# maxjaritz/mvpnet

Measured on AMD Instinct MI355X. Metric: chunks/sec (8192 pts, 3x160x120 views) fwd+bwd, higher is better.
Workload: dtype f32; 1 GPU; configs[2]: MVPNet lifting (unproject + pixel k-NN + gather) + FeatureAggregation + PN2SSG full train step (fwd+loss+bwd+Adam), 2D CNN replaced by a resident 64-ch feature map; cfg=mvpnet_3d_unet_resnet34_pn2ssg.yaml, chunks_per_gpu=32, points=8192, views=3x160x120, feature_channels=64, k=3, parallelism=dp1 (one process per GPU, 1 grad all-reduce/step), launch=eager, cpu_affinity=32 logical cpus of 256 (0 .. 183)

## Files before the change

mvpnet_amd/csrc/rows.hip:

```cpp
#include <algorithm>
#include "common.h"
#include "stats_reduce.h"
#include "dropout.h"

namespace {

constexpr int kRT = 256;

__device__ __forceinline__ float4 ld4(const float* p) { return *reinterpret_cast<const float4*>(p); }
__device__ __forceinline__ void st4(float* p, float4 v) { *reinterpret_cast<float4*>(p) = v; }

__global__ __launch_bounds__(kRT) void group_rows_kernel(const float* __restrict__ feat, const float* __restrict__ xyz,
                                                         const float* __restrict__ center,
                                                         const int64_t* __restrict__ idx, int N, int C, int M, int K,
                                                         int ld, float* __restrict__ out) {
  const int b = blockIdx.y;
  const int L4 = ld >> 2;
  const int64_t E = (int64_t)M * K;
  const int64_t t = (int64_t)blockIdx.x * kRT + threadIdx.x;
  const int64_t e = t / L4;
  const int c4 = (int)(t - e * L4);
  if (e >= E) return;
  const int64_t j = idx[(size_t)b * E + e];
  const bool ok = j >= 0 && j < N;
  const int c = c4 * 4;
  float4 v = make_float4(0.f, 0.f, 0.f, 0.f);
  if (c + 4 <= C) {
    if (ok) v = ld4(feat + ((size_t)b * N + j) * C + c);
  } else if (xyz && ok) {
    const int m = (int)(e / K);
    const float* p = xyz + ((size_t)b * N + j) * 3;
    const float* q = center + ((size_t)b * M + m) * 3;
    float r[4] = {0.f, 0.f, 0.f, 0.f};
#pragma unroll
    for (int i = 0; i < 4; ++i) {
      const int col = c + i - C;
      if (col >= 0 && col < 3) r[i] = p[col] - q[col];
    }
    v = make_float4(r[0], r[1], r[2], r[3]);
  }
  st4(out + ((size_t)b * E + e) * ld + c, v);
}

constexpr int kRelU = 4;
__global__ __launch_bounds__(kRT) void relation_rows_kernel(const float* __restrict__ feat, const float* __restrict__ src,
                                                            const float* __restrict__ tgt, int64_t rows, int K, int C,
                                                            float* __restrict__ out) {
  const int L4 = (C >> 2) + 1;
  const int64_t total = rows * L4;
  const int64_t t0 = (int64_t)blockIdx.x * (kRT * kRelU) + threadIdx.x;
  float4 v[kRelU];
  int64_t dst[kRelU];
#pragma unroll
  for (int u = 0; u < kRelU; ++u) {
    const int64_t t = t0 + (int64_t)u * kRT;
    dst[u] = -1;
    if (t < total) {
      const int64_t e = t / L4;
      const int c4 = (int)(t - e * L4);
      dst[u] = e * (C + 4) + c4 * 4;
      if (c4 < L4 - 1) {
        v[u] = ld4(feat + (size_t)e * C + c4 * 4);
      } else {
        const float* p = src + (size_t)e * 3;
        const float* q = tgt + (size_t)(e / K) * 3;
        const float dx = p[0] - q[0], dy = p[1] - q[1], dz = p[2] - q[2];
        v[u] = make_float4(dx, dy, dz, (dx * dx + dy * dy) + dz * dz);
      }
    }
  }
#pragma unroll
  for (int u = 0; u < kRelU; ++u)
    if (dst[u] >= 0) st4(out + dst[u], v[u]);
}

__global__ __launch_bounds__(kRT) void relation4_rows_kernel(const float* __restrict__ src, const float* __restrict__ tgt, int64_t rows, int K,
                                                             float* __restrict__ out) {
  const int64_t e = (int64_t)blockIdx.x * kRT + threadIdx.x;
  if (e >= rows) return;
  const float* p = src + (size_t)e * 3;
  const float* q = tgt + (size_t)(e / K) * 3;
  const float dx = p[0] - q[0], dy = p[1] - q[1], dz = p[2] - q[2];
  st4(out + (size_t)e * 4, make_float4(dx, dy, dz, (dx * dx + dy * dy) + dz * dz));
// ... 476 lines not shown
    const float *mm = p.mm, *ii = p.ii, *gm = p.gg, *bt = p.bb;
    float fo[4], go[4];
#pragma unroll
    for (int i = 0; i < 4; ++i) {
      const float dz = (!relu || oo[i] > 0.f) ? dd[i] : 0.f;
      float xh;
      if (fabsf(gm[i]) >= 0.05f * (1.0f + fabsf(bt[i])))
        xh = (oo[i] - bt[i]) / gm[i];
      else
        xh = (y[((size_t)g * K + a[i]) * C + c + i] - mm[i]) * ii[i];
      fo[i] = dz;
      go[i] = dz * xh;
    }
    f = make_float4(fo[0], fo[1], fo[2], fo[3]);
    gg = make_float4(go[0], go[1], go[2], go[3]);
  }
};

struct BwdMaxSel {
  const float *dout, *out, *ysel, *mean, *invstd;
  int relu;
  struct Params { float mm[4], ii[4]; };
  __device__ __forceinline__ Params params(int c) const {
    const float4 mu = ld4(mean + c), is = ld4(invstd + c);
    Params p;
    p.mm[0] = mu.x; p.mm[1] = mu.y; p.mm[2] = mu.z; p.mm[3] = mu.w;
    p.ii[0] = is.x; p.ii[1] = is.y; p.ii[2] = is.z; p.ii[3] = is.w;
    return p;
  }
  __device__ __forceinline__ void at(const Params& p, int64_t g, int c, int C, float4& f, float4& gg) const {
    const float4 d = ld4(dout + (size_t)g * C + c), o = ld4(out + (size_t)g * C + c), ys = ld4(ysel + (size_t)g * C + c);
    const float dd[4] = {d.x, d.y, d.z, d.w}, oo[4] = {o.x, o.y, o.z, o.w}, yy[4] = {ys.x, ys.y, ys.z, ys.w};
    float fo[4], go[4];
#pragma unroll
    for (int i = 0; i < 4; ++i) {
      const float dz = (!relu || oo[i] > 0.f) ? dd[i] : 0.f;
      fo[i] = dz;
      go[i] = dz * ((yy[i] - p.mm[i]) * p.ii[i]);
    }
    f = make_float4(fo[0], fo[1], fo[2], fo[3]);
    gg = make_float4(go[0], go[1], go[2], go[3]);
  }
};

__global__ __launch_bounds__(kRT) void pool_finalize_kernel(const float* __restrict__ ymax, const float* __restrict__ ymin,
                                                            const uint8_t* __restrict__ amax, const uint8_t* __restrict__ amin,
                                                            const float* __restrict__ mean, const float* __restrict__ invstd,
                                                            const float* __restrict__ gamma, const float* __restrict__ beta, int64_t G,
                                                            int C, int relu, float* __restrict__ out, uint8_t* __restrict__ arg,
                                                            float* __restrict__ ysel) {
  const int C4 = C >> 2;
  const int64_t t = (int64_t)blockIdx.x * kRT + threadIdx.x;
  const int64_t g = t / C4;
  const int c = (int)(t - g * C4) * 4;
  if (g >= G) return;
  const float4 mu = ld4(mean + c), is = ld4(invstd + c), ga = ld4(gamma + c), be = ld4(beta + c);
  const float4 hi = ld4(ymax + (size_t)g * C + c), lo = ld4(ymin + (size_t)g * C + c);
  const uchar4 ah = *reinterpret_cast<const uchar4*>(amax + (size_t)g * C + c), al = *reinterpret_cast<const uchar4*>(amin + (size_t)g * C + c);
  const float mm[4] = {mu.x, mu.y, mu.z, mu.w}, ii[4] = {is.x, is.y, is.z, is.w}, gg[4] = {ga.x, ga.y, ga.z, ga.w};
  const float bb[4] = {be.x, be.y, be.z, be.w}, hv[4] = {hi.x, hi.y, hi.z, hi.w}, lv[4] = {lo.x, lo.y, lo.z, lo.w};
  const uint8_t ha[4] = {ah.x, ah.y, ah.z, ah.w}, la[4] = {al.x, al.y, al.z, al.w};
  float o[4], ys[4];
  uint8_t ar[4];
#pragma unroll
  for (int i = 0; i < 4; ++i) {
    const bool up = gg[i] * ii[i] >= 0.f;
    ys[i] = up ? hv[i] : lv[i];
    ar[i] = up ? ha[i] : la[i];
    const float a = ((ys[i] - mm[i]) * ii[i]) * gg[i] + bb[i];
    o[i] = (relu && !(a > 0.f)) ? 0.f : a;
  }
  st4(out + (size_t)g * C + c, make_float4(o[0], o[1], o[2], o[3]));
  st4(ysel + (size_t)g * C + c, make_float4(ys[0], ys[1], ys[2], ys[3]));
  uchar4 u;
  u.x = ar[0]; u.y = ar[1]; u.z = ar[2]; u.w = ar[3];
  *reinterpret_cast<uchar4*>(arg + (size_t)g * C + c) = u;
}

struct BwdSum {
  const float *dout, *y, *mean, *invstd, *gamma, *beta;
  int K, relu;
  typedef ColParams Params;
  __device__ __forceinline__ Params params(int c) const { return load_col_params(mean, invstd, gamma, beta, c); }
  __device__ __forceinline__ void at(const Params& p, int64_t r, int c, int C, float4& f, float4& g) const {
    const float4 yy = ld4(y + (size_t)r * C + c), d = ld4(dout + (size_t)(r / K) * C + c);
    const float yv[4] = {yy.x, yy.y, yy.z, yy.w}, dd[4] = {d.x, d.y, d.z, d.w};
    float fo[4], go[4];
#pragma unroll
    for (int i = 0; i < 4; ++i) {
      const float xh = (yv[i] - p.mm[i]) * p.ii[i];
      const float dz = (!relu || xh * p.gg[i] + p.bb[i] > 0.f) ? dd[i] : 0.f;
      fo[i] = dz;
      go[i] = dz * xh;
    }
    f = make_float4(fo[0], fo[1], fo[2], fo[3]);
    g = make_float4(go[0], go[1], go[2], go[3]);
  }
};

template <typename Src>
__global__ __launch_bounds__(kRT) void colstats_kernel(Src src, int64_t R, int C, double* __restrict__ stat,
                                                       double* __restrict__ partial, int zero_stat) {
  if (zero_stat && blockIdx.x == 0)
    for (int j = threadIdx.x; j < 2 * C; j += kRT) stat[j] = 0.0;
  __shared__ double red[2][kRT][4];
  const int C4 = C >> 2;
  const int rpp = kRT / C4;
  const int c4 = threadIdx.x % C4, rg = threadIdx.x / C4;
  const int c = c4 * 4;
  const int64_t stride = (int64_t)gridDim.x * rpp;
  double ds[4] = {0, 0, 0, 0}, dq[4] = {0, 0, 0, 0};
  if (rg < rpp) {
    const typename Src::Params prm = src.params(c);
    int64_t r = (int64_t)blockIdx.x * rpp + rg;
    while (r < R) {
      float4 s = make_float4(0.f, 0.f, 0.f, 0.f), q = s;
      for (int it = 0; it < 16 && r < R; ++it, r += 4 * stride) {
        float4 f[4], g[4];
#pragma unroll
        for (int u = 0; u < 4; ++u) {
          f[u] = make_float4(0.f, 0.f, 0.f, 0.f);
          g[u] = f[u];
          if (r + u * stride < R) src.at(prm, r + u * stride, c, C, f[u], g[u]);
        }
#pragma unroll
        for (int u = 0; u < 4; ++u) {
          s.x += f[u].x; s.y += f[u].y; s.z += f[u].z; s.w += f[u].w;
          q.x += g[u].x; q.y += g[u].y; q.z += g[u].z; q.w += g[u].w;
        }
      }
      ds[0] += s.x; ds[1] += s.y; ds[2] += s.z; ds[3] += s.w;
      dq[0] += q.x; dq[1] += q.y; dq[2] += q.z; dq[3] += q.w;
    }
  }
  double* a = red[0][threadIdx.x];
  double* bq = red[1][threadIdx.x];
#pragma unroll
  for (int i = 0; i < 4; ++i) {
    a[i] = ds[i];
    bq[i] = dq[i];
  }
  __syncthreads();
  if (rg == 0) {
    double ts[4] = {0, 0, 0, 0}, tq[4] = {0, 0, 0, 0};
    for (int g = 0; g < rpp; ++g)
#pragma unroll
      for (int i = 0; i < 4; ++i) {
        ts[i] += red[0][g * C4 + c4][i];
        tq[i] += red[1][g * C4 + c4][i];
      }
    if (partial) {
      double* slot = partial + (size_t)blockIdx.x * 2 * C;
#pragma unroll
      for (int i = 0; i < 4; ++i) {
        slot[c + i] = ts[i];
        slot[C + c + i] = tq[i];
      }
    } else {
#pragma unroll
      for (int i = 0; i < 4; ++i) {
        atomicAdd(stat + c + i, ts[i]);
        atomicAdd(stat + C + c + i, tq[i]);
      }
    }
  }
}

__global__ void bn_finalize_kernel(const double* __restrict__ stat, int64_t R, int C, float eps, float momentum,
                                   float* __restrict__ mean, float* __restrict__ invstd,
                                   float* __restrict__ running_mean, float* __restrict__ running_var,
                                   int64_t* __restrict__ num_batches_tracked) {
  const int c = blockIdx.x * blockDim.x + threadIdx.x;
  if (c >= C) return;
  if (c == 0 && num_batches_tracked) *num_batches_tracked += 1;
  const double m = stat[c] / (double)R;
  double var = stat[C + c] / (double)R - m * m;
  if (var < 0.0) var = 0.0;
  mean[c] = (float)m;
  invstd[c] = (float)(1.0 / sqrt(var + (double)eps));
  if (running_mean) {
    const double unbiased = R > 1 ? var * ((double)R / (double)(R - 1)) : var;
    running_mean[c] = (float)((1.0 - momentum) * (double)running_mean[c] + momentum * m);
    running_var[c] = (float)((1.0 - momentum) * (double)running_var[c] + momentum * unbiased);
  }
}

template <bool RELU>
__global__ __launch_bounds__(kRT) void bn_act_kernel(const float* __restrict__ y, const float* __restrict__ mean,
                                                     const float* __restrict__ invstd, const float* __restrict__ gamma,
                                                     const float* __restrict__ beta, int64_t G, int K, int C,
                                                     float* __restrict__ out, uint8_t* __restrict__ arg) {
  const int C4 = C >> 2;
  const int64_t t = (int64_t)blockIdx.x * kRT + threadIdx.x;
  const int64_t g = t / C4;
  const int c = (int)(t - g * C4) * 4;
  if (g >= G) return;
  const float4 mu = ld4(mean + c), is = ld4(invstd + c), ga = ld4(gamma + c), be = ld4(beta + c);
  const bool sum = K > 1 && arg == nullptr;
  float best[4] = {-INFINITY, -INFINITY, -INFINITY, -INFINITY};
  if (sum) best[0] = best[1] = best[2] = best[3] = 0.f;
  int bk[4] = {0, 0, 0, 0};
  for (int k = 0; k < K; ++k) {
    const float4 yy = ld4(y + ((size_t)g * K + k) * C + c);
    float a[4] = {((yy.x - mu.x) * is.x) * ga.x + be.x, ((yy.y - mu.y) * is.y) * ga.y + be.y,
                  ((yy.z - mu.z) * is.z) * ga.z + be.z, ((yy.w - mu.w) * is.w) * ga.w + be.w};
#pragma unroll
    for (int i = 0; i < 4; ++i) {
      if (RELU) a[i] = a[i] > 0.f ? a[i] : 0.f;
      if (sum) {
        best[i] += a[i];
      } else if (a[i] > best[i]) {
        best[i] = a[i];
        bk[i] = k;
      }
    }
  }
  st4(out + (size_t)g * C + c, make_float4(best[0], best[1], best[2], best[3]));
  if (arg) {
    uchar4 u;
    u.x = (uint8_t)bk[0]; u.y = (uint8_t)bk[1]; u.z = (uint8_t)bk[2]; u.w = (uint8_t)bk[3];
    *reinterpret_cast<uchar4*>(arg + (size_t)g * C + c) = u;
  }
}

template <bool RELU>
__global__ __launch_bounds__(kRT) void bn_act_rows_kernel(const float* __restrict__ y, const float* __restrict__ mean,
                                                          const float* __restrict__ invstd, const float* __restrict__ gamma,
                                                          const float* __restrict__ beta, int64_t R, int C, float* __restrict__ out,
                                                          Dropout drop) {
  const int C4 = C >> 2;
  const int64_t t = (int64_t)blockIdx.x * kRT + threadIdx.x;
  const int64_t rg = t / C4;
  const int c = (int)(t - rg * C4) * 4;
  const int64_t r0 = rg * 8;
  if (r0 >= R) return;
  const float4 mu = ld4(mean + c), is = ld4(invstd + c), ga = ld4(gamma + c), be = ld4(beta + c);
#pragma unroll
  for (int h = 0; h < 8; h += 4) {
    float4 yy[4];
#pragma unroll
    for (int u = 0; u < 4; ++u) yy[u] = (r0 + h + u < R) ? ld4(y + (size_t)(r0 + h + u) * C + c) : make_float4(0.f, 0.f, 0.f, 0.f);
#pragma unroll
    for (int u = 0; u < 4; ++u) {
      if (r0 + h + u >= R) break;
      float a[4] = {((yy[u].x - mu.x) * is.x) * ga.x + be.x, ((yy[u].y - mu.y) * is.y) * ga.y + be.y,
                    ((yy[u].z - mu.z) * is.z) * ga.z + be.z, ((yy[u].w - mu.w) * is.w) * ga.w + be.w};
      if (RELU) {
#pragma unroll
        for (int i = 0; i < 4; ++i) a[i] = a[i] > 0.f ? a[i] : 0.f;
      }
      if (drop.thresh) {
        const unsigned e = (unsigned)((r0 + h + u) * C + c);
#pragma unroll
        for (int i = 0; i < 4; ++i) a[i] *= drop.factor(e + i);
      }
      st4(out + (size_t)(r0 + h + u) * C + c, make_float4(a[0], a[1], a[2], a[3]));
    }
  }
}

constexpr int kBwdRows = 8;
template <bool RELU>
__global__ __launch_bounds__(kRT) void bn_rows_bwd_kernel(const float* __restrict__ dsrc, const float* __restrict__ y,
                                                          const float* __restrict__ mean, const float* __restrict__ invstd,
                                                          const float* __restrict__ gamma, const float* __restrict__ beta,
                                                          const double* __restrict__ stat, int64_t R, int C, int batch_terms,
                                                          float* __restrict__ dy, float* __restrict__ dgamma,
                                                          float* __restrict__ dbeta, Dropout drop) {
  const int C4 = C >> 2;
  if (blockIdx.x == 0 && dgamma)
    for (int j = threadIdx.x; j < C; j += kRT) {
      dbeta[j] = (float)stat[j];
      dgamma[j] = (float)stat[C + j];
    }
  const int64_t t = (int64_t)blockIdx.x * kRT + threadIdx.x;
  const int64_t rg = t / C4;
  const int c = (int)(t - rg * C4) * 4;
  const int64_t r0 = rg * kBwdRows;
  if (r0 >= R) return;
  const float4 mu = ld4(mean + c), is = ld4(invstd + c), ga = ld4(gamma + c), be = ld4(beta + c);
  const float mm[4] = {mu.x, mu.y, mu.z, mu.w}, ii[4] = {is.x, is.y, is.z, is.w};
  const float gg[4] = {ga.x, ga.y, ga.z, ga.w}, bb[4] = {be.x, be.y, be.z, be.w};
  const float invR = batch_terms ? 1.0f / (float)R : 0.f;
  float sc[4], db[4], dg[4];
#pragma unroll
  for (int i = 0; i < 4; ++i) {
    sc[i] = gg[i] * ii[i];
    db[i] = (float)stat[c + i] * invR;
    dg[i] = (float)stat[C + c + i] * invR;
  }
#pragma unroll
  for (int h = 0; h < kBwdRows; h += 4) {
    float4 yy[4], dd[4];
#pragma unroll
    for (int u = 0; u < 4; ++u) {
      const int64_t r = r0 + h + u;
// ... 577 lines not shown
```

mvpnet_amd/csrc/sa_train.hip:

```cpp
#include "sa_common.h"
#include "stats_reduce.h"
#include <algorithm>
#include <stdlib.h>

namespace {

struct SaSrc {
  const float* zf;
  const float* xyz;
  const float* centre;
  const int64_t* index;
  const float* wxyz;
  const float* bn1[4];
  int64_t G;
  int N, M, C1;
};

template <int C1B>
__device__ __forceinline__ void stage_layer1(const SaSrc& p, float* P1 , float (*Wx)[4], int tid) {
  for (int k = tid; k < C1B * 32; k += kFT) {
    const int kc = min(k, p.C1 - 1);
#pragma unroll
    for (int a = 0; a < 4; ++a) P1[a * (C1B * 32) + k] = p.bn1[a] ? p.bn1[a][kc] : 0.f;
    Wx[k][0] = k < p.C1 ? p.wxyz[k * 3 + 0] : 0.f;
// ... 800 lines not shown
  }
  __shared__ unsigned last;
  wait_vm_complete();
  __syncthreads();
  unsigned* ticket = reinterpret_cast<unsigned*>(p.stat + 2 * C1);
  if (threadIdx.x == 0) last = atomicAdd(ticket, 1u) == gridDim.x - 1 ? 1u : 0u;
  __syncthreads();
  if (!last) return;
  const BnFinalize& fin = p.fin;
  if (p.rep) {
    for (int e = threadIdx.x; e < 5 * C1; e += 256) {
      double t = 0.0;
      for (int r = 0; r < p.nrep; ++r) t += __hip_atomic_load(p.rep + (size_t)r * 5 * C1 + e, __ATOMIC_RELAXED, __HIP_MEMORY_SCOPE_AGENT);
      if (e < 2 * C1) __hip_atomic_store(p.stat + e, t, __ATOMIC_RELAXED, __HIP_MEMORY_SCOPE_AGENT);
      else p.zsum[e - 2 * C1] = t;
    }
    __syncthreads();
  }
  for (int col = threadIdx.x; col < C1; col += 256) {
    const double s1 = __hip_atomic_load(p.stat + col, __ATOMIC_RELAXED, __HIP_MEMORY_SCOPE_AGENT);
    const double s2 = __hip_atomic_load(p.stat + C1 + col, __ATOMIC_RELAXED, __HIP_MEMORY_SCOPE_AGENT);
    const double m = s1 / (double)fin.rows;
    double var = s2 / (double)fin.rows - m * m;
    if (var < 0.0) var = 0.0;
    fin.mean[col] = (float)m;
    fin.invstd[col] = (float)(1.0 / sqrt(var + (double)fin.eps));
    if (fin.running_mean) {
      const double unbiased = fin.rows > 1 ? var * ((double)fin.rows / (double)(fin.rows - 1)) : var;
      fin.running_mean[col] = (float)((1.0 - fin.momentum) * (double)fin.running_mean[col] + fin.momentum * m);
      fin.running_var[col] = (float)((1.0 - fin.momentum) * (double)fin.running_var[col] + fin.momentum * unbiased);
    }
  }
  if (threadIdx.x == 0) {
    if (fin.num_batches_tracked) *fin.num_batches_tracked += 1;
    *ticket = 0u;
  }
}

struct SaBwd1Args {
  const float* dz1;
  const int* offsets;
  const int* slots;
  const float* zf;
  const float4* dsum;
  const float* wxyz;
  const float* mean;
  const float* invstd;
  const float* gamma;
  const double* stat;
  const float* tsum;
  const double* zsum;
  const double* gsum;
  float inv_rows;
  float* dgamma;
  float* dbeta;
  float* gz;
  float* dWx;
  int lddw;
  int B, N, M, C1;
};

__global__ __launch_bounds__(256) void sa_train_bwd1_kernel(SaBwd1Args p) {
  const int C1 = p.C1, C4 = C1 >> 2;
  if (blockIdx.x == 0 && blockIdx.y == 0) {
    const double* S = p.gsum;
    for (int t = threadIdx.x; t < C1 * 3; t += 256) {
      const int col = t / 3, k = t - col * 3;
      const double is = p.invstd[col], sc = (double)p.gamma[col] * is, mu = p.mean[col];
      const double db = p.stat[col] * (double)p.inv_rows, dg = p.stat[C1 + col] * (double)p.inv_rows;
      const double w0 = p.wxyz[col * 3 + 0], w1 = p.wxyz[col * 3 + 1], w2 = p.wxyz[col * 3 + 2];
      const double s2k0 = k == 0 ? S[3] : k == 1 ? S[4] : S[5], s2k1 = k == 0 ? S[4] : k == 1 ? S[6] : S[7], s2k2 = k == 0 ? S[5] : k == 1 ? S[7] : S[8];
      const double q = is * (p.zsum[col * 3 + k] + (w0 * s2k0 + w1 * s2k1 + w2 * s2k2) - mu * S[k]);
      double T = 0.0;
      for (int slot = 0; slot < 16; ++slot) T += (double)p.tsum[(size_t)slot * C1 * 4 + col * 4 + k];
      const double g = sc * ((T - db * S[k]) - dg * q);
      p.dWx[(size_t)col * p.lddw + k] += (float)g;
    }
    if (p.dgamma)
      for (int col = threadIdx.x; col < C1; col += 256) {
        p.dbeta[col] = (float)p.stat[col];
        p.dgamma[col] = (float)p.stat[C1 + col];
      }
  }
  const int b = blockIdx.y;
  const int64_t t = (int64_t)blockIdx.x * 256 + threadIdx.x;
  const int64_t j = t / C4;
  const int c = (int)(t - j * C4) * 4;
  if (j >= p.N) return;
  const int64_t E = (int64_t)p.M * 32;
  const int* o = p.offsets + (size_t)b * (p.N + 1) + j;
  const int p0 = o[0], p1 = o[1];
  const int* sl = p.slots + (size_t)b * E;
  const float* g = p.dz1 + (size_t)b * E * C1;
  float4 acc = make_float4(0.f, 0.f, 0.f, 0.f);
  int q = p0;
  for (; q + 3 < p1; q += 4) {
    int e[4];
#pragma unroll
    for (int u = 0; u < 4; ++u) e[u] = sl[q + u];
    float4 a[4];
#pragma unroll
    for (int u = 0; u < 4; ++u) a[u] = *reinterpret_cast<const float4*>(g + (size_t)e[u] * C1 + c);
#pragma unroll
    for (int u = 0; u < 4; ++u) {
      acc.x += a[u].x; acc.y += a[u].y; acc.z += a[u].z; acc.w += a[u].w;
    }
  }
  for (; q < p1; ++q) {
    const float4 a = *reinterpret_cast<const float4*>(g + (size_t)sl[q] * C1 + c);
    acc.x += a.x; acc.y += a.y; acc.z += a.z; acc.w += a.w;
  }
  const size_t pt = (size_t)b * p.N + j;
  const float4 z4 = *reinterpret_cast<const float4*>(p.zf + pt * C1 + c);
  const float4 d = p.dsum[pt];
  const float A[4] = {acc.x, acc.y, acc.z, acc.w}, z[4] = {z4.x, z4.y, z4.z, z4.w};
  float out[4];
#pragma unroll
  for (int i = 0; i < 4; ++i) {
    const int col = c + i;
    const float is = p.invstd[col], sc = p.gamma[col] * is, mu = p.mean[col];
    const float db = (float)p.stat[col] * p.inv_rows, dg = (float)p.stat[C1 + col] * p.inv_rows;
    const float wd = (p.wxyz[col * 3 + 0] * d.x + p.wxyz[col * 3 + 1] * d.y) + p.wxyz[col * 3 + 2] * d.z;
    const float xs = is * (d.w * (z[i] - mu) + wd);
    out[i] = sc * ((A[i] - d.w * db) - dg * xs);
  }
  *reinterpret_cast<float4*>(p.gz + pt * C1 + c) = make_float4(out[0], out[1], out[2], out[3]);
}

int blocks_of(int64_t c) { return c <= 32 ? 1 : c <= 64 ? 2 : 4; }

bool level_supported(int64_t K, int64_t C1, int64_t C2, int64_t C3) {
  return K == 32 && C1 >= 4 && C1 <= 64 && C2 <= 64 && C3 <= 128 && C1 % 4 == 0 && C2 % 4 == 0 && C3 % 4 == 0;
}

int64_t grid_for(int64_t G, int64_t lds_bytes, int64_t* tiles_per_wg, int64_t max_per_cu = 4) {
  const int64_t per_cu = std::max<int64_t>(1, std::min<int64_t>(max_per_cu, (150 * 1024) / lds_bytes));
  const int64_t wgs = std::max<int64_t>(1, std::min<int64_t>(std::min<int64_t>(1024, 256 * per_cu), cdiv(G, 16)));
  *tiles_per_wg = cdiv(cdiv(G, wgs), 4) * 4;
  return cdiv(G, *tiles_per_wg);
}

}

MVP_API int mvp_sa_train_forward_f32(int stage, const float* zf, const float* xyz, const float* centre, const int64_t* index, const float* wxyz,
                                     int64_t B, int64_t N, int64_t M, int64_t K, int64_t C1, const float* bn1_mean, const float* bn1_invstd,
                                     const float* bn1_gamma, const float* bn1_beta, const float* W2, int64_t C2, const float* bn2_mean,
                                     const float* bn2_invstd, const float* bn2_gamma, const float* bn2_beta, const float* W3, int64_t C3,
                                     double* stat, float eps, float momentum, float* mean, float* invstd, float* running_mean,
                                     float* running_var, int64_t* num_batches_tracked, float* ymax, float* ymin, uint8_t* amax,
                                     uint8_t* amin, mvp_stream_t stream) {
  MVP_NONNULL(zf);
  MVP_NONNULL(xyz);
  MVP_NONNULL(centre);
  MVP_NONNULL(index);
  MVP_NONNULL(wxyz);
  MVP_NONNULL(bn1_mean);
  MVP_NONNULL(bn1_invstd);
  MVP_NONNULL(bn1_gamma);
  MVP_NONNULL(bn1_beta);
  MVP_NONNULL(W2);
  MVP_NONNULL(stat);
  MVP_NONNULL(mean);
  MVP_NONNULL(invstd);
  MVP_REQUIRE(stage == 2 || stage == 3);
  MVP_REQUIRE(B >= 0 && N > 0 && M >= 0 && K > 0 && C1 > 0 && C2 > 0);
  if (stage == 3) {
    MVP_NONNULL(bn2_mean);
    MVP_NONNULL(bn2_invstd);
    MVP_NONNULL(bn2_gamma);
    MVP_NONNULL(bn2_beta);
    MVP_NONNULL(W3);
    MVP_NONNULL(ymax);
    MVP_NONNULL(ymin);
    MVP_NONNULL(amax);
    MVP_NONNULL(amin);
    MVP_REQUIRE(C3 > 0);
  }
  const int ns = mlp_fwd_pieces();
  if (ns == 0 || !level_supported(K, C1, C2, stage == 3 ? C3 : 4) || ((uintptr_t)zf % 16) != 0) return MVP_EUNSUPPORTED;
  if (B == 0 || M == 0) return MVP_OK;
  SaFwdArgs a;
  a.s.zf = zf; a.s.xyz = xyz; a.s.centre = centre; a.s.index = index; a.s.wxyz = wxyz;
  a.s.bn1[0] = bn1_mean; a.s.bn1[1] = bn1_invstd; a.s.bn1[2] = bn1_gamma; a.s.bn1[3] = bn1_beta;
  a.s.G = B * M; a.s.N = (int)N; a.s.M = (int)M; a.s.C1 = (int)C1;
  a.W2 = W2; a.C2 = (int)C2; a.W3 = W3; a.C3 = (int)(stage == 3 ? C3 : 0);
  a.bn2[0] = bn2_mean; a.bn2[1] = bn2_invstd; a.bn2[2] = bn2_gamma; a.bn2[3] = bn2_beta;
  a.stat = stat;
  a.fin = BnFinalize{B * M * K, eps, momentum, mean, invstd, running_mean, running_var, num_batches_tracked};
  a.ymax = ymax; a.ymin = ymin; a.amax = amax; a.amin = amin;
  const int c1b = blocks_of(C1), c2b = blocks_of(C2), c3b = stage == 3 ? blocks_of(C3) : 1;
  const int64_t lds = (int64_t)ns * 2048 * (c1b * c2b + (stage == 3 ? c2b * c3b : 0)) + 32 * 1024;
  const unsigned grid = (unsigned)grid_for(a.s.G, lds, &a.tiles_per_wg);
  hipStream_t s = static_cast<hipStream_t>(stream);
#define MVP_SAF(A_, B_, C_, ST_)                                                                                     \
  do {                                                                                                               \
    if (ns == 1) hipLaunchKernelGGL((sa_train_fwd_kernel<A_, B_, C_, 1, ST_>), dim3(grid), dim3(kFT), 0, s, a);       \
    else if (ns == 2) hipLaunchKernelGGL((sa_train_fwd_kernel<A_, B_, C_, 2, ST_>), dim3(grid), dim3(kFT), 0, s, a);  \
    else hipLaunchKernelGGL((sa_train_fwd_kernel<A_, B_, C_, 3, ST_>), dim3(grid), dim3(kFT), 0, s, a);               \
  } while (0)
  const int key = c1b * 100 + c2b * 10 + c3b;
  if (stage == 2) {
    switch (c1b * 10 + c2b) {
      case 11: MVP_SAF(1, 1, 1, 2); break;
      case 12: MVP_SAF(1, 2, 1, 2); break;
      case 21: MVP_SAF(2, 1, 1, 2); break;
// ... 106 lines not shown
      case 211: MVP_SAB(2, 1, 1, 3); break;
      case 212: MVP_SAB(2, 1, 2, 3); break;
      case 221: MVP_SAB(2, 2, 1, 3); break;
      case 222: MVP_SAB(2, 2, 2, 3); break;
      case 224: MVP_SAB(2, 2, 4, 3); break;
      default: return MVP_EUNSUPPORTED;
    }
  }
#undef MVP_SAB
  return mvp_launch_status();
}

MVP_API int mvp_sa_geom_sums_f32(const int32_t* offsets, const int32_t* slots, const float* xyz, const float* centre, int64_t B, int64_t N,
                                 int64_t M, int64_t K, float* dsum, double* gsum, mvp_stream_t stream) {
  MVP_NONNULL(offsets);
  MVP_NONNULL(slots);
  MVP_NONNULL(xyz);
  MVP_NONNULL(centre);
  MVP_NONNULL(dsum);
  MVP_NONNULL(gsum);
  MVP_REQUIRE(B >= 0 && N > 0 && M >= 0);
  if (K != 32 || ((uintptr_t)dsum % 16) != 0) return MVP_EUNSUPPORTED;
  if (B == 0) return MVP_OK;
  const unsigned grid = (unsigned)std::max<int64_t>(1, std::min<int64_t>(1024, cdiv(B * N, 256)));
  hipLaunchKernelGGL(sa_geom_sums_kernel, dim3(grid), dim3(256), 0, static_cast<hipStream_t>(stream), offsets, slots, xyz, centre, (int)B, (int)N,
                     (int)M, reinterpret_cast<float4*>(dsum), gsum);
  return mvp_launch_status();
}

MVP_API int mvp_sa_train_stats1_ws_f32(const float* zf, const float* dsum, const float* wxyz, const double* gsum, int64_t B, int64_t N, int64_t M,
                                       int64_t K, int64_t C1, double* stat, double* zsum, float eps, float momentum, float* mean, float* invstd,
                                       float* running_mean, float* running_var, int64_t* num_batches_tracked, double* scratch,
                                       int64_t scratch_doubles, mvp_stream_t stream) {
  MVP_NONNULL(zf);
  MVP_NONNULL(dsum);
  MVP_NONNULL(wxyz);
  MVP_NONNULL(gsum);
  MVP_NONNULL(stat);
  MVP_NONNULL(zsum);
  MVP_NONNULL(mean);
  MVP_NONNULL(invstd);
  MVP_REQUIRE(B >= 0 && N > 0 && M >= 0 && K > 0 && C1 > 0);
  if (C1 % 4 != 0 || C1 > 1024 || 256 % (C1 / 4) != 0 || ((uintptr_t)zf % 16) != 0 || ((uintptr_t)dsum % 16) != 0) return MVP_EUNSUPPORTED;
  if (B == 0 || M == 0) return MVP_OK;
  MVP_REQUIRE(scratch_doubles >= 0 && (scratch != nullptr || scratch_doubles == 0));
  const int nrep = scratch ? (int)std::min<int64_t>(16, scratch_doubles / (5 * C1)) : 0;
  SaStats1Args a{zf, reinterpret_cast<const float4*>(dsum), wxyz, gsum, stat, zsum, nrep >= 2 ? scratch : nullptr, nrep,
                 BnFinalize{B * M * K, eps, momentum, mean, invstd, running_mean, running_var, num_batches_tracked}, B * N, (int)C1};
  const int64_t ppw = 256 / (C1 / 4);
  static const int wgs = []() { const char* e = getenv("MVP_SA_STATS1_WGS"); return e ? atoi(e) : 256; }();
  const unsigned grid = (unsigned)std::max<int64_t>(1, std::min<int64_t>(wgs, cdiv(B * N, ppw * 8)));
  hipLaunchKernelGGL(sa_train_stats1_kernel, dim3(grid), dim3(256), 0, static_cast<hipStream_t>(stream), a);
  return mvp_launch_status();
}

MVP_API int mvp_sa_train_stats1_f32(const float* zf, const float* dsum, const float* wxyz, const double* gsum, int64_t B, int64_t N, int64_t M,
                                    int64_t K, int64_t C1, double* stat, double* zsum, float eps, float momentum, float* mean, float* invstd,
                                    float* running_mean, float* running_var, int64_t* num_batches_tracked, mvp_stream_t stream) {
  return mvp_sa_train_stats1_ws_f32(zf, dsum, wxyz, gsum, B, N, M, K, C1, stat, zsum, eps, momentum, mean, invstd, running_mean, running_var,
                                    num_batches_tracked, nullptr, 0, stream);
}

MVP_API int mvp_sa_train_backward1_f32(const float* dz1, const int32_t* offsets, const int32_t* slots, const float* zf, const float* dsum,
                                       const float* wxyz, const float* tsum, const double* zsum, const double* gsum, int64_t B, int64_t N,
                                       int64_t M, int64_t K, int64_t C1, const float* mean, const float* invstd, const float* gamma,
                                       const double* stat, int training, float* dgamma, float* dbeta, float* gz, float* dWxyz, int64_t lddw,
                                       mvp_stream_t stream) {
  MVP_NONNULL(dz1);
  MVP_NONNULL(offsets);
  MVP_NONNULL(slots);
  MVP_NONNULL(zf);
  MVP_NONNULL(dsum);
  MVP_NONNULL(wxyz);
  MVP_NONNULL(tsum);
  MVP_NONNULL(zsum);
  MVP_NONNULL(gsum);
  MVP_NONNULL(mean);
  MVP_NONNULL(invstd);
  MVP_NONNULL(gamma);
  MVP_NONNULL(stat);
  MVP_NONNULL(gz);
  MVP_NONNULL(dWxyz);
  MVP_REQUIRE(B >= 0 && B < 65536 && N > 0 && M >= 0 && C1 > 0 && lddw >= 3);
  if (K != 32 || C1 % 4 != 0 || ((uintptr_t)zf % 16) != 0 || ((uintptr_t)dsum % 16) != 0 || ((uintptr_t)dz1 % 16) != 0) return MVP_EUNSUPPORTED;
  if (B == 0) return MVP_OK;
  SaBwd1Args a{dz1, offsets, slots, zf, reinterpret_cast<const float4*>(dsum), wxyz, mean, invstd, gamma, stat, tsum, zsum, gsum,
               training ? 1.0f / (float)(B * M * K) : 0.f, dbeta ? dgamma : nullptr, dbeta, gz, dWxyz, (int)lddw, (int)B, (int)N, (int)M, (int)C1};
  hipLaunchKernelGGL(sa_train_bwd1_kernel, dim3((unsigned)cdiv(N * (C1 / 4), 256), (unsigned)B), dim3(256), 0, static_cast<hipStream_t>(stream), a);
  return mvp_launch_status();
}
```

mvpnet_amd/csrc/stats_reduce.h:

```cpp
#pragma once
#include "common.h"

namespace {

__global__ __launch_bounds__(256) void stats_reduce_kernel(const double* __restrict__ partial, int64_t nblk, int C2,
                                                           double* __restrict__ stat) {
  __shared__ double red[256];
  const int64_t per = (nblk + gridDim.x - 1) / gridDim.x;
  const int64_t t0 = (int64_t)blockIdx.x * per, t1 = min(nblk, t0 + per);
  const int cpp = min(C2, 256);
  const int phases = 256 / cpp;
  const int col = threadIdx.x % cpp, ph = threadIdx.x / cpp;
  for (int cb = 0; cb < C2; cb += cpp) {
    const int c = cb + col;
    double a0 = 0.0, a1 = 0.0, a2 = 0.0, a3 = 0.0;
    if (ph < phases && c < C2) {
      int64_t t = t0 + ph;
      for (; t + 3 * phases < t1; t += 4 * phases) {
        a0 += partial[(size_t)t * C2 + c];
        a1 += partial[(size_t)(t + phases) * C2 + c];
        a2 += partial[(size_t)(t + 2 * phases) * C2 + c];
        a3 += partial[(size_t)(t + 3 * phases) * C2 + c];
      }
      for (; t < t1; t += phases) a0 += partial[(size_t)t * C2 + c];
    }
    red[threadIdx.x] = (a0 + a1) + (a2 + a3);
    __syncthreads();
    if (ph == 0 && c < C2 && t1 > t0) {
      double acc = 0.0;
      for (int g = 0; g < phases; ++g) acc += red[g * cpp + col];
      atomicAdd(stat + c, acc);
    }
    __syncthreads();
  }
}


struct BnFinalize {
  int64_t rows;
  float eps, momentum;
  float* mean;
  float* invstd;
  float* running_mean;
  float* running_var;
  int64_t* num_batches_tracked;
};

__global__ __launch_bounds__(256) void stats_reduce_finalize_kernel(const double* __restrict__ partial, int64_t nblk, int C2,
                                                                    double* __restrict__ stat, BnFinalize fin) {
  __shared__ double red[256];
  __shared__ unsigned last;
  const int64_t per = (nblk + gridDim.x - 1) / gridDim.x;
  const int64_t t0 = (int64_t)blockIdx.x * per, t1 = min(nblk, t0 + per);
  const int cpp = min(C2, 256);
  const int phases = 256 / cpp;
  const int col = threadIdx.x % cpp, ph = threadIdx.x / cpp;
  for (int cb = 0; cb < C2; cb += cpp) {
    const int c = cb + col;
    double a0 = 0.0, a1 = 0.0, a2 = 0.0, a3 = 0.0;
    if (ph < phases && c < C2) {
      int64_t t = t0 + ph;
      for (; t + 3 * phases < t1; t += 4 * phases) {
        a0 += partial[(size_t)t * C2 + c];
        a1 += partial[(size_t)(t + phases) * C2 + c];
        a2 += partial[(size_t)(t + 2 * phases) * C2 + c];
        a3 += partial[(size_t)(t + 3 * phases) * C2 + c];
      }
      for (; t < t1; t += phases) a0 += partial[(size_t)t * C2 + c];
    }
    red[threadIdx.x] = (a0 + a1) + (a2 + a3);
    __syncthreads();
    if (ph == 0 && c < C2 && t1 > t0) {
      double acc = 0.0;
      for (int g = 0; g < phases; ++g) acc += red[g * cpp + col];
      atomicAdd(stat + c, acc);
    }
    __syncthreads();
  }
  wait_vm_complete();
  __syncthreads();
  unsigned* ticket = reinterpret_cast<unsigned*>(stat + C2);
  if (threadIdx.x == 0) last = atomicAdd(ticket, 1u) == gridDim.x - 1 ? 1u : 0u;
  __syncthreads();
  if (!last) return;
  const int C = C2 / 2;
  for (int c = threadIdx.x; c < C; c += 256) {
    const double s1 = __hip_atomic_load(stat + c, __ATOMIC_RELAXED, __HIP_MEMORY_SCOPE_AGENT);
    const double s2 = __hip_atomic_load(stat + C + c, __ATOMIC_RELAXED, __HIP_MEMORY_SCOPE_AGENT);
    const double m = s1 / (double)fin.rows;
    double var = s2 / (double)fin.rows - m * m;
    if (var < 0.0) var = 0.0;
    fin.mean[c] = (float)m;
    fin.invstd[c] = (float)(1.0 / sqrt(var + (double)fin.eps));
    if (fin.running_mean) {
      const double unbiased = fin.rows > 1 ? var * ((double)fin.rows / (double)(fin.rows - 1)) : var;
      fin.running_mean[c] = (float)((1.0 - fin.momentum) * (double)fin.running_mean[c] + fin.momentum * m);
      fin.running_var[c] = (float)((1.0 - fin.momentum) * (double)fin.running_var[c] + fin.momentum * unbiased);
    }
  }
  if (threadIdx.x == 0) {
    if (fin.num_batches_tracked) *fin.num_batches_tracked += 1;
    *ticket = 0u;
  }
}

static inline void launch_stats_reduce_finalize(const double* partial, int64_t nblk, int C2, double* stat, const BnFinalize& fin, hipStream_t s) {
  const int64_t blocks = nblk < 16 ? 1 : (nblk / 16 > 128 ? 128 : nblk / 16);
  hipLaunchKernelGGL(stats_reduce_finalize_kernel, dim3((unsigned)blocks), dim3(256), 0, s, partial, nblk, C2, stat, fin);
}

static inline void launch_stats_reduce(const double* partial, int64_t nblk, int C2, double* stat, hipStream_t s) {
  const int64_t blocks = nblk < 16 ? 1 : (nblk / 16 > 128 ? 128 : nblk / 16);
  hipLaunchKernelGGL(stats_reduce_kernel, dim3((unsigned)blocks), dim3(256), 0, s, partial, nblk, C2, stat);
}

}
```

Baseline: 5075 chunks/s.

## Restructure BN backward reductions, stats reduce grid, and SA bwd1 gather for more loads in flight

Several kernels are changed to raise memory-level parallelism. The BN backward column-stats path now walks groups directly, with a K=3 specialisation that reuses each dout load across the K rows. bn_act batches up to 8 row loads per iteration. The stats reduce kernel spreads column blocks over a 2D grid with 8-way unrolled loads. The SA bwd1 kernel stages per-column constants in shared memory and gathers 8 slots at a time. The cost is more registers and dynamic shared memory, plus a new C1<=1024 limit for bwd1.

```diff
diff --git a/mvpnet_amd/csrc/rows.hip b/mvpnet_amd/csrc/rows.hip
--- a/mvpnet_amd/csrc/rows.hip
+++ b/mvpnet_amd/csrc/rows.hip
@@ -1,4 +1,5 @@
 #include <algorithm>
+#include <type_traits>
 #include "common.h"
 #include "stats_reduce.h"
 #include "dropout.h"
@@ -641,8 +642,7 @@
   int K, relu;
   typedef ColParams Params;
   __device__ __forceinline__ Params params(int c) const { return load_col_params(mean, invstd, gamma, beta, c); }
-  __device__ __forceinline__ void at(const Params& p, int64_t r, int c, int C, float4& f, float4& g) const {
-    const float4 yy = ld4(y + (size_t)r * C + c), d = ld4(dout + (size_t)(r / K) * C + c);
+  __device__ __forceinline__ void add(const Params& p, const float4& yy, const float4& d, float4& s, float4& q) const {
     const float yv[4] = {yy.x, yy.y, yy.z, yy.w}, dd[4] = {d.x, d.y, d.z, d.w};
     float fo[4], go[4];
 #pragma unroll
@@ -652,8 +652,60 @@
       fo[i] = dz;
       go[i] = dz * xh;
     }
-    f = make_float4(fo[0], fo[1], fo[2], fo[3]);
-    g = make_float4(go[0], go[1], go[2], go[3]);
+    s.x += fo[0]; s.y += fo[1]; s.z += fo[2]; s.w += fo[3];
+    q.x += go[0]; q.y += go[1]; q.z += go[2]; q.w += go[3];
+  }
+  __device__ __forceinline__ void walk(const Params& p, int64_t G, int C, int c, int64_t g0, int64_t stride, double* ds, double* dq) const {
+    const float4 zero = make_float4(0.f, 0.f, 0.f, 0.f);
+    const float *yc = y + c, *dc = dout + c;
+    float4 s = zero, q = zero;
+    auto carry = [&]() {
+      ds[0] += s.x; ds[1] += s.y; ds[2] += s.z; ds[3] += s.w;
+      dq[0] += q.x; dq[1] += q.y; dq[2] += q.z; dq[3] += q.w;
+      s = zero;
+      q = zero;
+    };
+    int64_t g = g0;
+    if (K == 3) {
+      while (g < G) {
+        for (int it = 0; it < 10 && g < G; ++it, g += 2 * stride) {
+          const bool two = g + stride < G;
+          const float *ya = yc + (size_t)g * 3 * C, *yb = yc + (size_t)(g + stride) * 3 * C;
+          const float4 d0 = ld4(dc + (size_t)g * C), d1 = two ? ld4(dc + (size_t)(g + stride) * C) : zero;
+          const float4 a0 = ld4(ya), a1 = ld4(ya + C), a2 = ld4(ya + 2 * (size_t)C);
+          const float4 b0 = two ? ld4(yb) : zero, b1 = two ? ld4(yb + C) : zero, b2 = two ? ld4(yb + 2 * (size_t)C) : zero;
+          add(p, a0, d0, s, q);
+          add(p, a1, d0, s, q);
+          add(p, a2, d0, s, q);
+          if (two) {
+            add(p, b0, d1, s, q);
+            add(p, b1, d1, s, q);
+            add(p, b2, d1, s, q);
+          }
+        }
+        carry();
+      }
+      return;
+    }
+    int run = 0;
+    for (; g < G; g += stride) {
+      const float4 d = ld4(dc + (size_t)g * C);
+      const float* yg = yc + (size_t)g * K * C;
+      for (int k0 = 0; k0 < K; k0 += 4) {
+        float4 yy[4];
+#pragma unroll
+        for (int u = 0; u < 4; ++u) yy[u] = k0 + u < K ? ld4(yg + (size_t)(k0 + u) * C) : zero;
+#pragma unroll
+        for (int u = 0; u < 4; ++u)
+          if (k0 + u < K) add(p, yy[u], d, s, q);
+        run += min(4, K - k0);
+        if (run > 60) {
+          carry();
+          run = 0;
+        }
+      }
+    }
+    carry();
   }
 };
 
@@ -672,6 +724,9 @@
   if (rg < rpp) {
     const typename Src::Params prm = src.params(c);
     int64_t r = (int64_t)blockIdx.x * rpp + rg;
+    if constexpr (std::is_same<Src, BwdSum>::value) {
+      src.walk(prm, R / src.K, C, c, r, stride, ds, dq);
+    } else
     while (r < R) {
       float4 s = make_float4(0.f, 0.f, 0.f, 0.f), q = s;
       for (int it = 0; it < 16 && r < R; ++it, r += 4 * stride) {
@@ -759,18 +814,25 @@
   float best[4] = {-INFINITY, -INFINITY, -INFINITY, -INFINITY};
   if (sum) best[0] = best[1] = best[2] = best[3] = 0.f;
   int bk[4] = {0, 0, 0, 0};
-  for (int k = 0; k < K; ++k) {
-    const float4 yy = ld4(y + ((size_t)g * K + k) * C + c);
-    float a[4] = {((yy.x - mu.x) * is.x) * ga.x + be.x, ((yy.y - mu.y) * is.y) * ga.y + be.y,
-                  ((yy.z - mu.z) * is.z) * ga.z + be.z, ((yy.w - mu.w) * is.w) * ga.w + be.w};
-#pragma unroll
-    for (int i = 0; i < 4; ++i) {
-      if (RELU) a[i] = a[i] > 0.f ? a[i] : 0.f;
-      if (sum) {
-        best[i] += a[i];
-      } else if (a[i] > best[i]) {
-        best[i] = a[i];
-        bk[i] = k;
+  const float* yg = y + (size_t)g * K * C + c;
+  for (int k0 = 0; k0 < K; k0 += 8) {
+    float4 yy[8];
+#pragma unroll
+    for (int u = 0; u < 8; ++u) yy[u] = k0 + u < K ? ld4(yg + (size_t)(k0 + u) * C) : make_float4(0.f, 0.f, 0.f, 0.f);
+#pragma unroll
+    for (int u = 0; u < 8; ++u) {
+      if (k0 + u >= K) break;
+      float a[4] = {((yy[u].x - mu.x) * is.x) * ga.x + be.x, ((yy[u].y - mu.y) * is.y) * ga.y + be.y,
+                    ((yy[u].z - mu.z) * is.z) * ga.z + be.z, ((yy[u].w - mu.w) * is.w) * ga.w + be.w};
+#pragma unroll
+      for (int i = 0; i < 4; ++i) {
+        if (RELU) a[i] = a[i] > 0.f ? a[i] : 0.f;
+        if (sum) {
+          best[i] += a[i];
+        } else if (a[i] > best[i]) {
+          best[i] = a[i];
+          bk[i] = k0 + u;
+        }
       }
     }
   }
diff --git a/mvpnet_amd/csrc/sa_train.hip b/mvpnet_amd/csrc/sa_train.hip
--- a/mvpnet_amd/csrc/sa_train.hip
+++ b/mvpnet_amd/csrc/sa_train.hip
@@ -906,45 +906,62 @@
         p.dgamma[col] = (float)p.stat[C1 + col];
       }
   }
+  extern __shared__ __attribute__((aligned(16))) float cst[];
+  for (int col = threadIdx.x; col < C1; col += 256) {
+    const float is = p.invstd[col];
+    cst[0 * C1 + col] = is;
+    cst[1 * C1 + col] = p.gamma[col] * is;
+    cst[2 * C1 + col] = p.mean[col];
+    cst[3 * C1 + col] = (float)p.stat[col] * p.inv_rows;
+    cst[4 * C1 + col] = (float)p.stat[C1 + col] * p.inv_rows;
+    cst[5 * C1 + col] = p.wxyz[col * 3 + 0];
+    cst[6 * C1 + col] = p.wxyz[col * 3 + 1];
+    cst[7 * C1 + col] = p.wxyz[col * 3 + 2];
+  }
+  __syncthreads();
   const int b = blockIdx.y;
   const int64_t t = (int64_t)blockIdx.x * 256 + threadIdx.x;
   const int64_t j = t / C4;
   const int c = (int)(t - j * C4) * 4;
   if (j >= p.N) return;
   const int64_t E = (int64_t)p.M * 32;
-  const int* o = p.offsets + (size_t)b * (p.N + 1) + j;
-  const int p0 = o[0], p1 = o[1];
-  const int* sl = p.slots + (size_t)b * E;
-  const float* g = p.dz1 + (size_t)b * E * C1;
-  float4 acc = make_float4(0.f, 0.f, 0.f, 0.f);
-  int q = p0;
-  for (; q + 3 < p1; q += 4) {
-    int e[4];
-#pragma unroll
-    for (int u = 0; u < 4; ++u) e[u] = sl[q + u];
-    float4 a[4];
-#pragma unroll
-    for (int u = 0; u < 4; ++u) a[u] = *reinterpret_cast<const float4*>(g + (size_t)e[u] * C1 + c);
-#pragma unroll
-    for (int u = 0; u < 4; ++u) {
-      acc.x += a[u].x; acc.y += a[u].y; acc.z += a[u].z; acc.w += a[u].w;
-    }
-  }
-  for (; q < p1; ++q) {
-    const float4 a = *reinterpret_cast<const float4*>(g + (size_t)sl[q] * C1 + c);
-    acc.x += a.x; acc.y += a.y; acc.z += a.z; acc.w += a.w;
-  }
+  int2 pp;
+  __builtin_memcpy(&pp, p.offsets + (size_t)b * (p.N + 1) + j, sizeof(pp));
+  const int p0 = pp.x, p1 = pp.y;
   const size_t pt = (size_t)b * p.N + j;
   const float4 z4 = *reinterpret_cast<const float4*>(p.zf + pt * C1 + c);
   const float4 d = p.dsum[pt];
+  const int* sl = p.slots + (size_t)b * E;
+  const float* g = p.dz1 + (size_t)b * E * C1 + c;
+  float4 acc = make_float4(0.f, 0.f, 0.f, 0.f);
+  for (int q = p0; q < p1; q += 8) {
+    int e[8];
+#pragma unroll
+    for (int u = 0; u < 8; ++u) e[u] = q + u < p1 ? sl[q + u] : -1;
+    float4 a[8];
+#pragma unroll
+    for (int u = 0; u < 8; ++u) {
+      a[u] = make_float4(0.f, 0.f, 0.f, 0.f);
+      if (e[u] >= 0) a[u] = *reinterpret_cast<const float4*>(g + (size_t)e[u] * C1);
+    }
+#pragma unroll
+    for (int u = 0; u < 8; ++u)
+      if (e[u] >= 0) {
+        acc.x += a[u].x; acc.y += a[u].y; acc.z += a[u].z; acc.w += a[u].w;
+      }
+  }
   const float A[4] = {acc.x, acc.y, acc.z, acc.w}, z[4] = {z4.x, z4.y, z4.z, z4.w};
+  float k8[8][4];
+#pragma unroll
+  for (int k = 0; k < 8; ++k) {
+    const float4 v = *reinterpret_cast<const float4*>(cst + k * C1 + c);
+    k8[k][0] = v.x; k8[k][1] = v.y; k8[k][2] = v.z; k8[k][3] = v.w;
+  }
   float out[4];
 #pragma unroll
   for (int i = 0; i < 4; ++i) {
-    const int col = c + i;
-    const float is = p.invstd[col], sc = p.gamma[col] * is, mu = p.mean[col];
-    const float db = (float)p.stat[col] * p.inv_rows, dg = (float)p.stat[C1 + col] * p.inv_rows;
-    const float wd = (p.wxyz[col * 3 + 0] * d.x + p.wxyz[col * 3 + 1] * d.y) + p.wxyz[col * 3 + 2] * d.z;
+    const float is = k8[0][i], sc = k8[1][i], mu = k8[2][i], db = k8[3][i], dg = k8[4][i];
+    const float wd = (k8[5][i] * d.x + k8[6][i] * d.y) + k8[7][i] * d.z;
     const float xs = is * (d.w * (z[i] - mu) + wd);
     out[i] = sc * ((A[i] - d.w * db) - dg * xs);
   }
@@ -1217,10 +1234,11 @@
   MVP_NONNULL(gz);
   MVP_NONNULL(dWxyz);
   MVP_REQUIRE(B >= 0 && B < 65536 && N > 0 && M >= 0 && C1 > 0 && lddw >= 3);
-  if (K != 32 || C1 % 4 != 0 || ((uintptr_t)zf % 16) != 0 || ((uintptr_t)dsum % 16) != 0 || ((uintptr_t)dz1 % 16) != 0) return MVP_EUNSUPPORTED;
+  if (K != 32 || C1 % 4 != 0 || C1 > 1024 || ((uintptr_t)zf % 16) != 0 || ((uintptr_t)dsum % 16) != 0 || ((uintptr_t)dz1 % 16) != 0) return MVP_EUNSUPPORTED;
   if (B == 0) return MVP_OK;
   SaBwd1Args a{dz1, offsets, slots, zf, reinterpret_cast<const float4*>(dsum), wxyz, mean, invstd, gamma, stat, tsum, zsum, gsum,
                training ? 1.0f / (float)(B * M * K) : 0.f, dbeta ? dgamma : nullptr, dbeta, gz, dWxyz, (int)lddw, (int)B, (int)N, (int)M, (int)C1};
-  hipLaunchKernelGGL(sa_train_bwd1_kernel, dim3((unsigned)cdiv(N * (C1 / 4), 256), (unsigned)B), dim3(256), 0, static_cast<hipStream_t>(stream), a);
+  hipLaunchKernelGGL(sa_train_bwd1_kernel, dim3((unsigned)cdiv(N * (C1 / 4), 256), (unsigned)B), dim3(256), 8 * C1 * sizeof(float),
+                     static_cast<hipStream_t>(stream), a);
   return mvp_launch_status();
 }
diff --git a/mvpnet_amd/csrc/stats_reduce.h b/mvpnet_amd/csrc/stats_reduce.h
--- a/mvpnet_amd/csrc/stats_reduce.h
+++ b/mvpnet_amd/csrc/stats_reduce.h
@@ -3,38 +3,47 @@
 
 namespace {
 
+constexpr int kSrLoads = 8;
+
+__device__ __forceinline__ void stats_reduce_block(const double* __restrict__ partial, int64_t nblk, int C2, double* __restrict__ stat,
+                                                   double* red) {
+  const int64_t per = (nblk + gridDim.y - 1) / gridDim.y;
+  const int64_t t0 = (int64_t)blockIdx.y * per, t1 = min(nblk, t0 + per);
+  const int cpp = min(C2, 256);
+  const int phases = 256 / cpp;
+  const int col = threadIdx.x % cpp, ph = threadIdx.x / cpp;
+  const int c = blockIdx.x * cpp + col;
+  double a[kSrLoads];
+#pragma unroll
+  for (int u = 0; u < kSrLoads; ++u) a[u] = 0.0;
+  if (ph < phases && c < C2) {
+    const double* pc = partial + c;
+    for (int64_t t = t0 + ph; t < t1; t += (int64_t)kSrLoads * phases) {
+      double v[kSrLoads];
+#pragma unroll
+      for (int u = 0; u < kSrLoads; ++u) v[u] = t + (int64_t)u * phases < t1 ? pc[(size_t)(t + (int64_t)u * phases) * C2] : 0.0;
+#pragma unroll
+      for (int u = 0; u < kSrLoads; ++u) a[u] += v[u];
+    }
+  }
+#pragma unroll
+  for (int w = kSrLoads / 2; w > 0; w >>= 1)
+#pragma unroll
+    for (int u = 0; u < w; ++u) a[u] += a[u + w];
+  red[threadIdx.x] = a[0];
+  __syncthreads();
+  if (ph == 0 && c < C2 && t1 > t0) {
+    double acc = 0.0;
+    for (int g = 0; g < phases; ++g) acc += red[g * cpp + col];
+    atomicAdd(stat + c, acc);
+  }
+}
+
 __global__ __launch_bounds__(256) void stats_reduce_kernel(const double* __restrict__ partial, int64_t nblk, int C2,
                                                            double* __restrict__ stat) {
   __shared__ double red[256];
-  const int64_t per = (nblk + gridDim.x - 1) / gridDim.x;
-  const int64_t t0 = (int64_t)blockIdx.x * per, t1 = min(nblk, t0 + per);
-  const int cpp = min(C2, 256);
-  const int phases = 256 / cpp;
-  const int col = threadIdx.x % cpp, ph = threadIdx.x / cpp;
-  for (int cb = 0; cb < C2; cb += cpp) {
-    const int c = cb + col;
-    double a0 = 0.0, a1 = 0.0, a2 = 0.0, a3 = 0.0;
-    if (ph < phases && c < C2) {
-      int64_t t = t0 + ph;
-      for (; t + 3 * phases < t1; t += 4 * phases) {
-        a0 += partial[(size_t)t * C2 + c];
-        a1 += partial[(size_t)(t + phases) * C2 + c];
-        a2 += partial[(size_t)(t + 2 * phases) * C2 + c];
-        a3 += partial[(size_t)(t + 3 * phases) * C2 + c];
-      }
-      for (; t < t1; t += phases) a0 += partial[(size_t)t * C2 + c];
-    }
-    red[threadIdx.x] = (a0 + a1) + (a2 + a3);
-    __syncthreads();
-    if (ph == 0 && c < C2 && t1 > t0) {
-      double acc = 0.0;
-      for (int g = 0; g < phases; ++g) acc += red[g * cpp + col];
-      atomicAdd(stat + c, acc);
-    }
-    __syncthreads();
-  }
+  stats_reduce_block(partial, nblk, C2, stat, red);
 }
-
 
 struct BnFinalize {
   int64_t rows;
@@ -50,37 +59,11 @@
                                                                     double* __restrict__ stat, BnFinalize fin) {
   __shared__ double red[256];
   __shared__ unsigned last;
-  const int64_t per = (nblk + gridDim.x - 1) / gridDim.x;
-  const int64_t t0 = (int64_t)blockIdx.x * per, t1 = min(nblk, t0 + per);
-  const int cpp = min(C2, 256);
-  const int phases = 256 / cpp;
-  const int col = threadIdx.x % cpp, ph = threadIdx.x / cpp;
-  for (int cb = 0; cb < C2; cb += cpp) {
-    const int c = cb + col;
-    double a0 = 0.0, a1 = 0.0, a2 = 0.0, a3 = 0.0;
-    if (ph < phases && c < C2) {
-      int64_t t = t0 + ph;
-      for (; t + 3 * phases < t1; t += 4 * phases) {
-        a0 += partial[(size_t)t * C2 + c];
-        a1 += partial[(size_t)(t + phases) * C2 + c];
-        a2 += partial[(size_t)(t + 2 * phases) * C2 + c];
-        a3 += partial[(size_t)(t + 3 * phases) * C2 + c];
-      }
-      for (; t < t1; t += phases) a0 += partial[(size_t)t * C2 + c];
-    }
-    red[threadIdx.x] = (a0 + a1) + (a2 + a3);
-    __syncthreads();
-    if (ph == 0 && c < C2 && t1 > t0) {
-      double acc = 0.0;
-      for (int g = 0; g < phases; ++g) acc += red[g * cpp + col];
-      atomicAdd(stat + c, acc);
-    }
-    __syncthreads();
-  }
+  stats_reduce_block(partial, nblk, C2, stat, red);
   wait_vm_complete();
   __syncthreads();
   unsigned* ticket = reinterpret_cast<unsigned*>(stat + C2);
-  if (threadIdx.x == 0) last = atomicAdd(ticket, 1u) == gridDim.x - 1 ? 1u : 0u;
+  if (threadIdx.x == 0) last = atomicAdd(ticket, 1u) == gridDim.x * gridDim.y - 1 ? 1u : 0u;
   __syncthreads();
   if (!last) return;
   const int C = C2 / 2;
@@ -104,14 +87,17 @@
   }
 }
 
+static inline dim3 stats_reduce_grid(int64_t nblk, int C2) {
+  const int64_t chunks = nblk < 16 ? 1 : (nblk / 16 > 128 ? 128 : nblk / 16);
+  return dim3((unsigned)((C2 + 255) / 256), (unsigned)chunks);
+}
+
 static inline void launch_stats_reduce_finalize(const double* partial, int64_t nblk, int C2, double* stat, const BnFinalize& fin, hipStream_t s) {
-  const int64_t blocks = nblk < 16 ? 1 : (nblk / 16 > 128 ? 128 : nblk / 16);
-  hipLaunchKernelGGL(stats_reduce_finalize_kernel, dim3((unsigned)blocks), dim3(256), 0, s, partial, nblk, C2, stat, fin);
+  hipLaunchKernelGGL(stats_reduce_finalize_kernel, stats_reduce_grid(nblk, C2), dim3(256), 0, s, partial, nblk, C2, stat, fin);
 }
 
 static inline void launch_stats_reduce(const double* partial, int64_t nblk, int C2, double* stat, hipStream_t s) {
-  const int64_t blocks = nblk < 16 ? 1 : (nblk / 16 > 128 ? 128 : nblk / 16);
-  hipLaunchKernelGGL(stats_reduce_kernel, dim3((unsigned)blocks), dim3(256), 0, s, partial, nblk, C2, stat);
+  hipLaunchKernelGGL(stats_reduce_kernel, stats_reduce_grid(nblk, C2), dim3(256), 0, s, partial, nblk, C2, stat);
 }
 
 }
```

New measurement: 5113 chunks/s (median of 4 runs). About the same (+0.8%).
